# jumerckx/Monodepth2.jl

Measured on AMD Instinct MI355X. Metric: train-step images/sec, ResNet-18 416×128; 1/2/4/8 MI355X + roofline %, higher is better.
Workload: dtype fp32; 1 GPU; train_step resnet18 depth+pose decoders, 4-scale photometric loss, ADAM; batch_per_gpu=12, global_batch=12, height=128, width=416, parallelism=dp1

## Files before the change

monodepth2.jl_amd/csrc/conv_impl.inc:

```
#include <type_traits>

#include "conv.h"
#include "head.h"

namespace md2 {

typedef float f32x16 __attribute__((ext_vector_type(16)));

constexpr int KPAD = 32;
constexpr int MPAD = 128;

static inline long round_up(long a, long b) { return (a + b - 1) / b * b; }

__device__ __forceinline__ int refl(int i, int n) { return i < 0 ? -i : (i >= n ? 2 * n - 2 - i : i); }

__device__ __forceinline__ float apply_act(float v, int act) {
  switch (act) {
    case ACT_RELU: return fmaxf(v, 0.f);
    case ACT_ELU: return v > 0.f ? v : expm1f(v);
    case ACT_SIGMOID: return 1.f / (1.f + expf(-v));
    default: return v;
  }
}

// ... 156 lines not shown
  }
}

__global__ __launch_bounds__(256) void pack_batch_kernel(const PackJob* __restrict__ jobs, int njobs) {
  __shared__ int s_job;
  if (threadIdx.x == 0) {
    int lo = 0, hi = njobs - 1;
    while (lo < hi) {
      const int mid = (lo + hi + 1) >> 1;
      if (jobs[mid].block_begin <= (long)blockIdx.x) lo = mid; else hi = mid - 1;
    }
    s_job = lo;
  }
  __syncthreads();
  const PackJob& j = jobs[__builtin_amdgcn_readfirstlane(s_job)];
  if (j.tiled) {
    pack_tile(j, (int)(blockIdx.x - j.block_begin));
    return;
  }
  const unsigned e = (unsigned)(blockIdx.x - j.block_begin) * 256u + threadIdx.x;
  const unsigned KK = (unsigned)j.KK, Cinw = (unsigned)j.Cinw;
  if (e >= (unsigned)j.Cout * Cinw * KK) return;
  const float v = j.w[e];
  const unsigned row = e / KK;
  const int tap = (int)(e - row * KK);
  const int co = (int)(row / Cinw);
  const int ci = (int)(row - (unsigned)co * Cinw);
  if (j.f.out) {
    const int k = j.f.tap ? tap * j.Cin + ci : ci * j.KK + tap;
    pack_store(j.f.out, k, co, j.f.layout, j.f.Mpad, v);
  }
  if (j.d.out) {
    const int k = j.d.tap ? tap * j.Cout + co : co * j.KK + tap;
    pack_store(j.d.out, k, ci, j.d.layout, j.d.Mpad, v);
  }
}

int& conv_arith_ref() {
  static thread_local int v = 1;
  return v;
}
int conv_last_arith() { return conv_arith_ref(); }

int conv_pack_batch(const PackJob* dev_jobs, int njobs, long total_blocks, hipStream_t st) {
  if (njobs == 0) return MD2_OK;
  hipLaunchKernelGGL(pack_batch_kernel, dim3(total_blocks), dim3(256), 0, st, dev_jobs, njobs);
  MD2_LAUNCH_CHECK();
  return MD2_OK;
}

#endif

struct GemmDims {
  int M;
  long N;
  int K;
  int kper;
  int Mpad;
};

struct ConvArgs {
  GemmDims g;
  int Cin, H, W, Cout, Ho, Wo, stride, pad;
  long HW, HoWo;
  FastDiv fd_pix;
  FastDiv fd_row;
  FastDiv fd_bdiv;
  TensorIn in;
  const float* A;
  const float* dy;
  TensorOut out;
  float* slab;
  uint32_t A_bytes, b0_bytes, b1_bytes;
  uint32_t HW4, HoWo4;
  int ph_y0, ph_x0;
  int ph_taps[16];
  int ph_S;
  int ph_y0c[4], ph_x0c[4], ph_ntc[4];
  int xcd;
  int hx_cper;
  int hx_r, hx_nchunk;
  int hx_ext;
  double* bn_part;
};

__device__ __forceinline__ void out_pixel(const ConvArgs& a, bool phase, int y0, int x0, long nn,
                                          int& img, long& pix, long& plane) {
  img = (int)fdiv((uint32_t)nn, a.fd_pix);
  const long r = nn - (long)img * a.fd_pix.d;
  if (phase) {
    const int jy = (int)fdiv((uint32_t)r, a.fd_row);
    const int jx = (int)(r - (long)jy * a.fd_row.d);
    pix = (long)(y0 + 2 * jy) * a.W + x0 + 2 * jx;
    plane = a.HW;
  } else {
    pix = r;
    plane = a.fd_pix.d;
  }
}

__device__ __forceinline__ void out_pixel(const ConvArgs& a, bool phase, long nn, int& img, long& pix,
                                          long& plane) {
  out_pixel(a, phase, a.ph_y0, a.ph_x0, nn, img, pix, plane);
}

template <int TM, int TN, int BK>
__device__ __forceinline__ void mma_chunk(const float* __restrict__ As, int lda,
                                          const float* __restrict__ Bs, int ldb, int am0, int bn0,
                                          int lane, f32x16 (&acc)[TM][TN]) {
  const int kh = lane >> 5, l = lane & 31;
  float a[2][TM], b[2][TN];
#pragma unroll
  for (int i = 0; i < TM; ++i) a[0][i] = As[kh * lda + am0 + i * 32 + l];
#pragma unroll
  for (int j = 0; j < TN; ++j) b[0][j] = Bs[kh * ldb + bn0 + j * 32 + l];
#pragma unroll
  for (int kk = 0; kk < BK / 2; ++kk) {
    const int cur = kk & 1, nxt = cur ^ 1;
    if (kk + 1 < BK / 2) {
#pragma unroll
      for (int i = 0; i < TM; ++i) a[nxt][i] = As[(2 * kk + 2 + kh) * lda + am0 + i * 32 + l];
#pragma unroll
      for (int j = 0; j < TN; ++j) b[nxt][j] = Bs[(2 * kk + 2 + kh) * ldb + bn0 + j * 32 + l];
    }
#pragma unroll
    for (int i = 0; i < TM; ++i)
#pragma unroll
      for (int j = 0; j < TN; ++j)
        acc[i][j] = __builtin_amdgcn_mfma_f32_32x32x2f32(a[cur][i], b[cur][j], acc[i][j], 0, 0, 0);
  }
}

__device__ __forceinline__ void store_out(const TensorOut& o, int m, int img, long pix, long HoWo,
                                          float v) {
  if (o.bias) v += o.bias[m];
  v = apply_act(v, o.act);
  float* dst = (m < o.c0) ? o.p0 + (long)img * o.bs0 + (long)m * HoWo + pix
                          : o.p1 + (long)img * o.bs1 + (long)(m - o.c0) * HoWo + pix;
  if (o.accumulate)
    *dst += v;
  else
    *dst = v;
}

#include "conv_px.inc"
#include "conv_px2.inc"
#include "conv_px16.inc"
#include "conv_px3.inc"
#include "conv_wpx3.inc"

constexpr int HX_PX = 736;
constexpr int HX_PLANE = HX_PX * 32;
constexpr int HX_PAD = 16;
constexpr int HS2_PX = 416;
constexpr int HS2_PLANE = HS2_PX * 32;
int halo_launch(int mode, const ConvArgs& a, int items, int splits, int reflect, hipStream_t st);
int halo2d_launch(int mode, const ConvArgs& a, int mw, int splits, int reflect, hipStream_t st);
int halo_s2_launch(const ConvArgs& a, int items, int splits, hipStream_t st);
int whalo_launch(const ConvArgs& a, int items, int ksteps, int splits, hipStream_t st);
int& conv_arith_ref();
bool stem_s2d_applies(const ConvShape& s, const TensorIn& x, const TensorOut& y);
int stem_s2d_launch(const ConvShape& s, const ConvArgs& a, hipStream_t st);
bool stem_wgrad_s2d_applies(const ConvShape& s, const TensorIn& x);
int stem_wgrad_blocks(const ConvShape& s);
int stem_wgrad_s2d_launch(const ConvShape& s, const ConvArgs& a, hipStream_t st);

template <int P_ = 0>
__global__ __launch_bounds__(256) void splitk_reduce_px4_kernel(ConvArgs a, int splits) {
  const long idx = 4 * ((long)blockIdx.x * 256 + threadIdx.x);
  const long total = (long)a.g.M * a.g.N;
  if (idx >= total) return;
  const int m = (int)(idx / a.g.N);
  const long nn = idx - (long)m * a.g.N;
  float4 v = make_float4(0.f, 0.f, 0.f, 0.f);
#pragma unroll 4
  for (int s = 0; s < splits; ++s) {
    const float4 t = *reinterpret_cast<const float4*>(a.slab + (long)s * total + idx);
    v.x += t.x; v.y += t.y; v.z += t.z; v.w += t.w;
  }
  const TensorOut& o = a.out;
  const int img = (int)fdiv((uint32_t)nn, a.fd_pix);
  const long pix = nn - (long)img * a.fd_pix.d, HoWo = a.fd_pix.d;
  float r[4] = {v.x, v.y, v.z, v.w};
#pragma unroll
  for (int q = 0; q < 4; ++q) {
    if (o.bias) r[q] += o.bias[m];
    r[q] = apply_act(r[q], o.act);
  }
  float* dst = (m < o.c0) ? o.p0 + (long)img * o.bs0 + (long)m * HoWo + pix
                          : o.p1 + (long)img * o.bs1 + (long)(m - o.c0) * HoWo + pix;
  float4 w = make_float4(r[0], r[1], r[2], r[3]);
  if (o.accumulate) {
    const float4 d = *reinterpret_cast<const float4*>(dst);
    w.x = d.x + w.x; w.y = d.y + w.y; w.z = d.z + w.z; w.w = d.w + w.w;
  }
  *reinterpret_cast<float4*>(dst) = w;
}

template <int P_ = 0>
__global__ __launch_bounds__(256) void splitk_reduce_px_kernel(ConvArgs a, int splits, int phase, FastDiv fdN,
                                                               FastDiv fdT) {
  uint32_t idx = blockIdx.x * 256u + threadIdx.x;
  const uint32_t total = fdT.d;
  int cls = 0, y0 = a.ph_y0, x0 = a.ph_x0;
  if (phase && a.ph_S > 0) {
    cls = (int)fdiv(idx, fdT);
    if (cls >= 4) return;
    idx -= (uint32_t)cls * total;
    y0 = a.ph_y0c[cls];
    x0 = a.ph_x0c[cls];
  } else if (idx >= total) {
    return;
  }
  const int m = (int)fdiv(idx, fdN);
  const uint32_t nn = idx - (uint32_t)m * fdN.d;
  const float* p = a.slab + (size_t)cls * splits * total + idx;
  float v = 0.f;
  int s = 0;
  for (; s + 3 < splits; s += 4) {
    const float t0 = p[(size_t)s * total], t1 = p[(size_t)(s + 1) * total];
    const float t2 = p[(size_t)(s + 2) * total], t3 = p[(size_t)(s + 3) * total];
    v += t0;
    v += t1;
    v += t2;
    v += t3;
  }
  for (; s < splits; ++s) v += p[(size_t)s * total];
  int img;
  long pix, plane;
  out_pixel(a, phase != 0, y0, x0, (long)nn, img, pix, plane);
  store_out(a.out, m, img, pix, plane, v);
}

template <bool SMALL>
__global__ __launch_bounds__(256) void fold_reflect_kernel(const float* __restrict__ src, int splits, long ss,
                                                           long sn, long sc, TensorOut o, FastDiv fd_hw,
                                                           FastDiv fd_w, FastDiv fd_c, uint32_t total) {
  constexpr int NR = SMALL ? 3 : 2;
  const uint32_t idx = blockIdx.x * 256u + threadIdx.x;
  if (idx >= total) return;
  const int H = (int)fd_hw.d / (int)fd_w.d, W = (int)fd_w.d, P = W + 2;
  const uint32_t nc = fdiv(idx, fd_hw);
// ... 640 lines not shown

namespace {

constexpr int TARGET_BLOCKS = 1536;

enum TileCfg { T128x128 = 0, T64x256 = 1, T32x256 = 2, T64x128 = 3, T128x64 = 4, T64x64 = 5, T32x128 = 6,
               T128x64q = 7 };
const int TILE_BM[] = {128, 64, 32, 64, 128, 64, 32, 128};
const int TILE_BN[] = {128, 256, 256, 128, 64, 64, 128, 64};

int env_int(const char* name, int dflt) { return tuning_knob(name, dflt); }

struct Plan {
  int tile;
  int BM, BN, BK;
  int splits;
  int kper;
};

Plan plan_px(int M, long N, int K, bool bk32_ok = false, bool prefer32 = false) {
  static const int tile_override = env_int("MD2_PX_TILE", -1);
  static const int target = env_int("MD2_PX_TARGET", TARGET_BLOCKS);
  Plan p{};
  p.tile = M > 32 ? T64x64 : T32x128;
  if (tile_override >= 0 && tile_override <= T128x64q &&
      ((M > 32 && TILE_BM[tile_override] >= 64) || (M <= 32 && TILE_BM[tile_override] == 32)))
    p.tile = tile_override;
  p.BM = TILE_BM[p.tile];
  p.BN = TILE_BN[p.tile];
  static const int bk_override = env_int("MD2_PX_BK", 0);
  p.BK = ((bk_override == 32 || (prefer32 && bk_override != 16)) && bk32_ok) ? 32 : 16;
  if (K <= 0) {
    p.splits = 1;
    p.kper = p.BK;
    return p;
  }
  static const int minch = std::max(1, env_int("MD2_PX_MINCH", 8));
  const long tiles = (long)cdiv(M, p.BM) * cdiv(N, p.BN);
  int splits = 1;
  while (tiles * splits * 2 <= target && K / (splits * 2) >= minch * p.BK) splits *= 2;
  p.kper = (int)round_up(cdiv(K, splits), p.BK);
  p.splits = cdiv(K, p.kper);
  return p;
}

struct HaloPlan {
  bool ok = false;
  int items = 0, splits = 1, cper = 1;
  bool d2 = false;
  int mw = 2;
};
HaloPlan plan_halo(const ConvShape& s, int mode) {
  HaloPlan h;
  static const int on = env_int("MD2_HALO", 1);
  static const int target = env_int("MD2_HX_TARGET", 256);
  if (!on || mode > 1 || s.KH != 3 || s.KW != 3 || s.stride != 1 || s.pad != 1 || (s.reflect && mode == 1)) return h;
  if (!conv_px3_used(s, mode) || !conv_tap_major(s, mode)) return h;
  const int M = mode == 0 ? s.Cout : s.Cin, C = mode == 0 ? s.Cin : s.Cout;
  if (C % 16 || s.cin_w) return h;
  const int hrmax = 255 / s.W + 4;
  const bool flat = M % 64 == 0 && hrmax * (s.W + HX_PAD) + 3 <= HX_PX && cdiv((long)hrmax * s.W, 512) <= 2;
  static const int d2on = env_int("MD2_HALO2D", 1);
  const bool d2 = !flat && (d2on >> mode & 1) && M % 32 == 0 && tuning_knob("MD2_PX3_TERMS", 6) != 9 &&
                  2L * s.H * s.W >= (long)round_up(s.H, 8) * round_up(s.W, 32);
  if (!flat && !d2) return h;
  long tiles;
  int tgt = target;
  if (flat) {
    h.items = cdiv((long)hrmax * s.W, 512);
    tiles = (long)(M / 64) * cdiv((long)s.N * s.H * s.W, 256);
  } else {
    h.d2 = true;
    h.mw = M % 64 == 0 ? 2 : 1;
    tiles = (long)(M / (32 * h.mw)) * s.N * cdiv(s.H, 8) * cdiv(s.W, 32);
    tgt = h.mw == 1 ? 2 * target : target;
  }
  const int nch = C / 16;
  int splits = 1;
  while (tiles * splits * 2 <= tgt && nch / (splits * 2) >= 2) splits *= 2;
  h.cper = cdiv(nch, splits);
  h.splits = cdiv(nch, h.cper);
  h.ok = true;
  return h;
}

struct HaloS2Plan {
  bool ok = false;
  int items = 0, splits = 1, cper = 1;
};
HaloS2Plan plan_halo_s2(const ConvShape& s) {
  HaloS2Plan h;
  static const int on = env_int("MD2_HALO_S2", 1);
  if (!on || s.KH != 3 || s.KW != 3 || s.stride != 2 || s.pad != 1 || s.reflect || s.cin_w) return h;
  if (s.H != 2 * s.Ho || s.W != 2 * s.Wo || s.Cin % 64 || s.Cout % 16) return h;
  if (!conv_px3_used(s, 1) || !conv_tap_major(s, 1) || tuning_knob("MD2_PX3_TERMS", 6) == 9) return h;
  const int hrmax = 127 / s.Wo + 4;
  if (hrmax * (s.Wo + HX_PAD) + 3 > HS2_PX) return h;
  h.items = 1;
  const long tiles = (long)(s.Cin / 64) * cdiv((long)s.N * s.Ho * s.Wo, 128);
  const int nch = s.Cout / 16;
  int splits = 1;
  while (tiles * splits * 2 <= 256 && nch / (splits * 2) >= 2) splits *= 2;
  h.cper = cdiv(nch, splits);
  h.splits = cdiv(nch, h.cper);
  h.ok = true;
  return h;
}

struct WHaloPlan {
  bool ok = false;
  int r = 0, items = 0, nchunk = 0, splits = 1, cper = 1;
};
WHaloPlan plan_whalo(const ConvShape& s, int c0) {
  WHaloPlan h;
  static const int on = env_int("MD2_WHALO", 1);
  static const int target = env_int("MD2_WHX_TARGET", 256);
  if (!on || s.KH != 3 || s.KW != 3 || s.stride != 1 || s.pad != 1 || s.reflect) return h;
  if (s.Cin % 32 || s.Cout % 64 || c0 < s.Cin || (s.cin_w && s.cin_w != s.Cin) || s.W > 112) return h;
  if (tuning_knob("MD2_PX3_TERMS", 6) == 9) return h;
  int r = 0;
  for (int d = 1; d <= s.H; ++d)
    if (s.H % d == 0 && d * s.W <= 112) r = d;
  if (r == 0 || (r * s.W) % 4 || (s.H * s.W) % 4 || r * s.W < 49) return h;
  if (3L * (((r + 2) * (s.W + 2) + 3) * 64) + 448 > 65536) return h;
  static const int maxit = env_int("MD2_WHX_MAXITEMS", 4);
  h.items = cdiv(4L * (r + 2) * s.W, 384);
  if (h.items > std::min(4, maxit)) return h;
  h.r = r;
  h.nchunk = s.N * s.H / r;
  const long tiles = (long)(s.Cin / 32) * (s.Cout / 64);
  long splits = std::max(1L, (long)target / tiles);
  splits = std::min(splits, std::max(1L, (long)h.nchunk / 2));
  h.cper = cdiv(h.nchunk, splits);
  h.splits = cdiv(h.nchunk, h.cper);
  h.ok = true;
  return h;
}

ConvShape reflect_ext_shape(const ConvShape& s) {
  ConvShape e = s;
  e.H = s.H + 2;
  e.W = s.W + 2;
  e.Ho = e.H;
  e.Wo = e.W;
  e.reflect = 0;
  return e;
}
bool reflect_dgrad_on_halo(const ConvShape& s, HaloPlan* hp = nullptr) {
  static const int on = env_int("MD2_HALO_RFL_DGRAD", 1);
  if (!on || !s.reflect || s.KH != 3 || s.stride != 1 || s.pad != 1 || s.cin_w || s.H < 2 || s.W < 2) return false;
  const HaloPlan h = plan_halo(reflect_ext_shape(s), 1);
  if (hp) *hp = h;
  return h.ok;
}
size_t reflect_dgrad_ws(const ConvShape& s) {
  HaloPlan h;
  if (!reflect_dgrad_on_halo(s, &h)) return 0;
  const long Ne = (long)s.N * (s.H + 2) * (s.W + 2);
  return ((size_t)(h.splits > 1 ? h.splits : 0) + 1) * s.Cin * Ne * sizeof(float);
}

enum WTileCfg { W64x128 = 0, W32x256 = 1, W64x64 = 2, W32x128 = 3, W16x144 = 4, WSTEM = 5, W64x192 = 6 };
const int WT_BM[] = {64, 32, 64, 32, 16, 64, 64};
const int WT_BN[] = {128, 256, 64, 128, 144, 64, 192};

struct WPlan {
// ... 101 lines not shown

int check_shape(const ConvShape& s) {
  MD2_CHECK_ARG(s.N > 0 && s.Cin > 0 && s.Cout > 0 && s.H > 0 && s.W > 0, "conv dims");
  MD2_CHECK_ARG(s.KH == s.KW && (s.KH == 1 || s.KH == 3 || s.KH == 7), "kernel size 1/3/7");
  MD2_CHECK_ARG(s.stride == 1 || s.stride == 2, "stride 1/2");
  MD2_CHECK_ARG(s.Ho == (s.H + 2 * s.pad - s.KH) / s.stride + 1 &&
                    s.Wo == (s.W + 2 * s.pad - s.KW) / s.stride + 1, "output size");
  MD2_CHECK_ARG(!s.reflect || (s.KH == 3 && s.stride == 1 && s.pad == 1 && s.H >= 2 && s.W >= 2),
                "reflect padding needs 3x3/1 pad 1");
  MD2_CHECK_ARG((long)s.N * s.H * s.W < (1L << 31) && (long)s.N * s.Ho * s.Wo < (1L << 31),
                "pixel count");
  MD2_CHECK_ARG(s.cin_w >= 0 && s.cin_w <= s.Cin && (s.cin_w == 0 || s.Cout > 1),
                "weight channels (cin_w) must be <= Cin (and no padded head convs)");
  return MD2_OK;
}

#define MD2_CONV_COMBOS(X) X(1, 1, 0) X(1, 2, 0) X(3, 1, 0) X(3, 1, 1) X(3, 2, 0) X(7, 2, 0)

static int px3_terms() {
  static const int t = tuning_knob("MD2_PX3_TERMS", 6) == 9 ? 9 : 6;
  return t;
}

template <int MODE, int BM, int BN, int WM, int WN>
int launch_px_tile(const ConvShape& s, const ConvArgs& a, bool tap, int bk, dim3 grid, hipStream_t st) {
  const bool v2 = conv_px2_used(s, MODE);
  const bool v3 = conv_px3_used(s, MODE);
#define MD2_PX_CASE(KS, SS, RR)                                                                  \
  if (s.KH == KS && s.stride == SS && s.reflect == RR) {                                         \
    if constexpr (BM >= 32 && BN % 64 == 0 && WM * WN == 4) {                                    \
      if (v3) {                                                                                  \
        conv_arith_ref() = 6;                                                                    \
        if (px3_terms() == 6)                                                                    \
          hipLaunchKernelGGL((conv_px3_kernel<MODE, BM, BN, WM, WN, KS, KS, SS, RR, 16, 6>), grid, \
                             dim3(256), 0, st, a);                                               \
        else                                                                                     \
          hipLaunchKernelGGL((conv_px3_kernel<MODE, BM, BN, WM, WN, KS, KS, SS, RR, 16, 9>), grid, \
                             dim3(256), 0, st, a);                                               \
        MD2_LAUNCH_CHECK();                                                                      \
        return MD2_OK;                                                                           \
      }                                                                                          \
    }                                                                                            \
    if constexpr (BM >= 64 && BN % 64 == 0) {                                                    \
      if (v2) {                                                                                  \
        conv_arith_ref() = 1;                                                                    \
        if (bk == 32)                                                                            \
          hipLaunchKernelGGL((conv_px2_kernel<MODE, BM, BN, WM, WN, KS, KS, SS, RR, 32>), grid,  \
                             dim3(256), 0, st, a);                                               \
        else                                                                                     \
          hipLaunchKernelGGL((conv_px2_kernel<MODE, BM, BN, WM, WN, KS, KS, SS, RR, 16>), grid,  \
                             dim3(256), 0, st, a);                                               \
        MD2_LAUNCH_CHECK();                                                                      \
        return MD2_OK;                                                                           \
      }                                                                                          \
    }                                                                                            \
    if (v2) {                                                                                    \
      set_error("conv: k-contiguous kernel needs a tile with BM >= 64");                         \
      return MD2_EINVAL;                                                                         \
    }                                                                                            \
    conv_arith_ref() = 1;                                                                        \
    if (tap && bk == 32)                                                                         \
      hipLaunchKernelGGL((conv_px_kernel<MODE, 1, BM, BN, 32, WM, WN, KS, KS, SS, RR>), grid,    \
                         dim3(256), 0, st, a);                                                   \
    else if (tap)                                                                                \
      hipLaunchKernelGGL((conv_px_kernel<MODE, 1, BM, BN, 16, WM, WN, KS, KS, SS, RR>), grid,    \
                         dim3(256), 0, st, a);                                                   \
    else                                                                                         \
      hipLaunchKernelGGL((conv_px_kernel<MODE, 0, BM, BN, 16, WM, WN, KS, KS, SS, RR>), grid,    \
                         dim3(256), 0, st, a);                                                   \
    MD2_LAUNCH_CHECK();                                                                          \
    return MD2_OK;                                                                               \
  }
  MD2_CONV_COMBOS(MD2_PX_CASE)
#undef MD2_PX_CASE
  set_error("conv: unsupported (kernel, stride, padding) combination");
  return MD2_ENOTSUP;
}

template <int MODE>
int launch_px16(const ConvShape& s, ConvArgs& a, hipStream_t st) {
  a.slab = nullptr;
  conv_arith_ref() = 1;
  a.g.kper = (int)round_up(a.g.K, 16);
  static const int bn = env_int("MD2_PX16_BN", 128);
  const bool big = bn == 256;
  const dim3 grid(cdiv(a.g.N, big ? 256 : 128));
#define MD2_P16_CASE(KS, SS, RR)                                                                 \
  if constexpr (SS == 1) {                                                                       \
    if (s.KH == KS && s.stride == SS && s.reflect == RR) {                                       \
      if (big)                                                                                   \
        hipLaunchKernelGGL((conv_px16_kernel<MODE, 256, KS, KS, SS, RR>), grid, dim3(256), 0, st, a); \
      else                                                                                       \
        hipLaunchKernelGGL((conv_px16_kernel<MODE, 128, KS, KS, SS, RR>), grid, dim3(256), 0, st, a); \
      MD2_LAUNCH_CHECK();                                                                        \
      return MD2_OK;                                                                             \
    }                                                                                            \
  }
  MD2_P16_CASE(3, 1, 0) MD2_P16_CASE(3, 1, 1)
#undef MD2_P16_CASE
  set_error("conv: 16-row kernel supports 3x3 stride 1 only");
  return MD2_ENOTSUP;
}

template <int MODE>
int launch_px(const ConvShape& s, ConvArgs& a, const Plan& p_in, ConvWorkspace ws, hipStream_t st,
              SplitKDefer* defer = nullptr) {
  double* const stats = defer ? defer->stats : nullptr;
  const bool keep_reduce = defer && defer->keep_reduce;
  if (defer) *defer = SplitKDefer{};
  if (conv_px16_used(s, MODE)) return launch_px16<MODE>(s, a, st);
  HaloPlan hp = plan_halo(s, MODE);
  if (hp.ok && MODE == 0 && (a.in.bdiv < s.N || (a.in.p1 && a.in.c0 < s.Cin && a.in.c0 % 16))) hp.ok = false;
  Plan p = p_in;
  if (hp.ok) {
    p.splits = hp.splits;
    p.kper = hp.cper * 16;
  }
  a.g.kper = p.kper;
  a.slab = nullptr;
  if (p.splits > 1) {
    const size_t need = (size_t)p.splits * a.g.M * a.g.N * sizeof(float);
    MD2_CHECK_ARG(ws.ptr && ws.bytes >= need, "conv split-K workspace too small");
    a.slab = (float*)ws.ptr;
  }
  const int ncls = (MODE == 1 && a.ph_S > 0) ? 4 : 1;
  if (ncls > 1) {
    a.ph_S = p.splits;
    MD2_CHECK_ARG(p.splits == 1 || (ws.ptr && ws.bytes >= 4 * (size_t)p.splits * a.g.M * a.g.N * sizeof(float)),
                  "conv split-K workspace too small");
  }
  dim3 grid(cdiv(a.g.N, p.BN), cdiv(a.g.M, p.BM), p.splits * ncls);
  const bool tap = conv_tap_major(s, MODE);
  int rc;
  if (hp.ok && ncls == 1) {
    a.hx_cper = hp.cper;
    const TensorOut& oo = a.out;
    const bool bnst = MODE == 0 && stats && !hp.d2 && hp.splits == 1 && !s.reflect && !oo.bias && oo.act == ACT_NONE &&
                      !oo.accumulate && oo.c0 >= a.g.M && oo.bs0 == (long)a.g.M * a.fd_pix.d;
    a.bn_part = bnst ? stats : nullptr;
    conv_arith_ref() = 6;
    rc = hp.d2 ? halo2d_launch(MODE, a, hp.mw, hp.splits, s.reflect, st)
               : halo_launch(MODE, a, hp.items, hp.splits, s.reflect, st);
    a.bn_part = nullptr;
    if (rc == MD2_OK && bnst) {
      defer->stats = stats;
      defer->stats_parts = (int)cdiv(a.g.N, 256);
    }
  } else switch (p.tile) {
    case T128x128: rc = launch_px_tile<MODE, 128, 128, 2, 2>(s, a, tap, p.BK, grid, st); break;
    case T64x256: rc = launch_px_tile<MODE, 64, 256, 1, 4>(s, a, tap, p.BK, grid, st); break;
    case T64x128: rc = launch_px_tile<MODE, 64, 128, 2, 2>(s, a, tap, p.BK, grid, st); break;
    case T128x64: rc = launch_px_tile<MODE, 128, 64, 2, 2>(s, a, tap, p.BK, grid, st); break;
    case T64x64: rc = launch_px_tile<MODE, 64, 64, 2, 2>(s, a, tap, p.BK, grid, st); break;
    case T32x128: rc = launch_px_tile<MODE, 32, 128, 1, 4>(s, a, tap, p.BK, grid, st); break;
    case T128x64q: rc = launch_px_tile<MODE, 128, 64, 4, 1>(s, a, tap, p.BK, grid, st); break;
    default: rc = launch_px_tile<MODE, 32, 256, 1, 4>(s, a, tap, p.BK, grid, st); break;
  }
  if (rc) return rc;
  const TensorOut& o = a.out;
  if (defer && !keep_reduce && p.splits > 1 && ncls == 1 && (MODE == 0 || s.stride == 1) && !o.bias && o.act == ACT_NONE &&
      !o.accumulate && o.c0 >= a.g.M && o.bs0 == (long)a.g.M * a.fd_pix.d) {
    defer->slab = a.slab;
    defer->splits = p.splits;
    return MD2_OK;
  }
  const int phase = (int)(MODE == 1 && s.stride == 2 && conv_tap_major(s, 1));
  const bool aligned4 = a.fd_pix.d % 4 == 0 && o.bs0 % 4 == 0 && (!o.p1 || o.bs1 % 4 == 0) &&
                        ((uintptr_t)o.p0 % 16) == 0 && (!o.p1 || ((uintptr_t)o.p1 % 16) == 0);
  if (p.splits > 1 && ncls == 1 && !phase && aligned4) {
    const long total4 = (long)a.g.M * a.g.N / 4;
    hipLaunchKernelGGL(splitk_reduce_px4_kernel<0>, dim3(cdiv(total4, 256)), dim3(256), 0, st, a,
                       p.splits);
    MD2_LAUNCH_CHECK();
    return MD2_OK;
  }
  if (p.splits > 1) {
    const long total = (long)a.g.M * a.g.N * ncls;
    MD2_CHECK_ARG(total < (1L << 31), "conv: split-K reduction index exceeds 2^31");
    hipLaunchKernelGGL(splitk_reduce_px_kernel<0>, dim3(cdiv(total, 256)), dim3(256), 0, st, a, p.splits,
                       (int)(MODE == 1 && s.stride == 2 && conv_tap_major(s, 1)),
                       make_fastdiv((uint32_t)a.g.N), make_fastdiv((uint32_t)((long)a.g.M * a.g.N)));
    MD2_LAUNCH_CHECK();
  }
  return MD2_OK;
}

static bool wgrad_px3_on() {
  static const int v = tuning_knob("MD2_WPX3", 1);
  return v != 0;
}

template <int BM, int BN, int WM, int WN, int KS, int SS, int RR, int CW, int PX>
// ... 553 lines not shown
    default: return g;
  }
}

__global__ __launch_bounds__(256) void act_bias_kernel(const float* __restrict__ out,
                                                       const float* __restrict__ dout,
                                                       float* __restrict__ dpre, int C, int parts,
                                                       uint32_t U, FastDiv fdq, int act,
                                                       float* __restrict__ part) {
  __shared__ float red[4];
  const int c = blockIdx.x, p = blockIdx.y;
  const uint32_t beg = (uint32_t)((unsigned long long)U * p / parts);
  const uint32_t end = (uint32_t)((unsigned long long)U * (p + 1) / parts);
  const uint32_t Q = fdq.d;
  float s = 0.f;
  constexpr int UN = 4;
  for (uint32_t u0 = beg + threadIdx.x; u0 < end; u0 += 256 * UN) {
    float4 o[UN], g[UN];
    long idx[UN];
#pragma unroll
    for (int q = 0; q < UN; ++q) {
      const uint32_t u = u0 + 256 * q;
      const uint32_t uu = u < end ? u : u0;
      const uint32_t img = fdiv(uu, fdq), k = uu - img * Q;
      idx[q] = ((long)(img * (uint32_t)C + (uint32_t)c) * Q + k) * 4;
      o[q] = *reinterpret_cast<const float4*>(out + idx[q]);
      g[q] = *reinterpret_cast<const float4*>(dout + idx[q]);
    }
#pragma unroll
    for (int q = 0; q < UN; ++q) {
      if (u0 + 256 * q >= end) break;
      float4 d;
      d.x = act_grad(o[q].x, g[q].x, act);
      d.y = act_grad(o[q].y, g[q].y, act);
      d.z = act_grad(o[q].z, g[q].z, act);
      d.w = act_grad(o[q].w, g[q].w, act);
      *reinterpret_cast<float4*>(dpre + idx[q]) = d;
      s += (d.x + d.y) + (d.z + d.w);
    }
  }
  float v[1] = {s};
  block_sum256<1>(v, red);
  if (threadIdx.x == 0) part[(long)c * parts + p] = v[0];
}

int act_bias_parts(int C, int N, long HW) {
  const long U = (long)N * HW / 4;
  return (int)std::max(1L, std::min((long)std::max(1, 2048 / C), U / 1024 + 1));
}

int act_backward_bias(const float* out, const float* dout, float* dpre, int N, int C, long HW,
                      int act, float* part, hipStream_t st) {
  MD2_CHECK_ARG(HW % 4 == 0 && (long)N * C * HW < (1L << 31), "act_backward_bias: HW % 4, size");
  const int parts = act_bias_parts(C, N, HW);
  hipLaunchKernelGGL(act_bias_kernel, dim3(C, parts), dim3(256), 0, st, out, dout, dpre, C, parts,
                     (uint32_t)((long)N * HW / 4), make_fastdiv((uint32_t)(HW / 4)), act, part);
  MD2_LAUNCH_CHECK();
  return MD2_OK;
}

int act_backward(const float* out, const float* dout, float* dpre, long n, int act,
                 hipStream_t st) {
  hipLaunchKernelGGL(act_backward_kernel, dim3(cdiv(n, 256)), dim3(256), 0, st, out, dout, dpre, n,
                     act);
  MD2_LAUNCH_CHECK();
  return MD2_OK;
}

#endif

}

#if MD2_CONV_PART == 4
namespace md2 {
#include "conv_halo.inc"
}
#endif

#if MD2_CONV_PART == 5
namespace md2 {
#include "conv_stem.inc"
}
#endif
```

Baseline: 1909 images/s.

## Add thin-channel 3x3 conv kernel with LDS halo tiles and split-bf16 MFMA

```diff
diff --git a/monodepth2.jl_amd/csrc/conv_impl.inc b/monodepth2.jl_amd/csrc/conv_impl.inc
--- a/monodepth2.jl_amd/csrc/conv_impl.inc
+++ b/monodepth2.jl_amd/csrc/conv_impl.inc
@@ -262,6 +262,7 @@
   int hx_r, hx_nchunk;
   int hx_ext;
   double* bn_part;
+  int thin_layout;
 };
 
 __device__ __forceinline__ void out_pixel(const ConvArgs& a, bool phase, int y0, int x0, long nn,
@@ -338,6 +339,8 @@
 int halo2d_launch(int mode, const ConvArgs& a, int mw, int splits, int reflect, hipStream_t st);
 int halo_s2_launch(const ConvArgs& a, int items, int splits, hipStream_t st);
 int whalo_launch(const ConvArgs& a, int items, int ksteps, int splits, hipStream_t st);
+int thin_launch(int mode, const ConvArgs& a, int mt, int nch, int reflect, hipStream_t st);
+size_t thin_lds_host(int mt, int nch);
 int& conv_arith_ref();
 bool stem_s2d_applies(const ConvShape& s, const TensorIn& x, const TensorOut& y);
 int stem_s2d_launch(const ConvShape& s, const ConvArgs& a, hipStream_t st);
@@ -1144,6 +1147,26 @@
   h.splits = cdiv(nch, h.cper);
   h.ok = true;
   return h;
+}
+
+struct ThinPlan {
+  bool ok = false;
+  int mt = 1, nch = 1, layout = 0;
+};
+ThinPlan plan_thin(const ConvShape& s, int mode) {
+  ThinPlan t;
+  static const int on = env_int("MD2_THIN", 3);
+  if (mode > 1 || !(on >> mode & 1) || s.KH != 3 || s.KW != 3 || s.stride != 1 || s.pad != 1 || s.cin_w) return t;
+  if (s.H < 2 || s.W < 2 || !conv_tap_major(s, mode)) return t;
+  const int M = mode == 0 ? s.Cout : s.Cin, C = mode == 0 ? s.Cin : s.Cout;
+  if ((M != 16 && M != 32) || (C != 16 && C != 32) || (M == 32 && C == 32)) return t;
+  if ((M == 32 || C == 32) && !(on & 4)) return t;
+  if (conv_px3_used(s, mode)) return t;
+  t.layout = (conv_px2_used(s, mode) || conv_px16_used(s, mode)) ? 1 : 0;
+  t.mt = M / 16;
+  t.nch = C / 16;
+  t.ok = true;
+  return t;
 }
 
 struct HaloS2Plan {
@@ -1411,16 +1434,11 @@
   a.slab = nullptr;
   conv_arith_ref() = 1;
   a.g.kper = (int)round_up(a.g.K, 16);
-  static const int bn = env_int("MD2_PX16_BN", 128);
-  const bool big = bn == 256;
-  const dim3 grid(cdiv(a.g.N, big ? 256 : 128));
+  const dim3 grid(cdiv(a.g.N, 128));
 #define MD2_P16_CASE(KS, SS, RR)                                                                 \
   if constexpr (SS == 1) {                                                                       \
     if (s.KH == KS && s.stride == SS && s.reflect == RR) {                                       \
-      if (big)                                                                                   \
-        hipLaunchKernelGGL((conv_px16_kernel<MODE, 256, KS, KS, SS, RR>), grid, dim3(256), 0, st, a); \
-      else                                                                                       \
-        hipLaunchKernelGGL((conv_px16_kernel<MODE, 128, KS, KS, SS, RR>), grid, dim3(256), 0, st, a); \
+      hipLaunchKernelGGL((conv_px16_kernel<MODE, 128, KS, KS, SS, RR>), grid, dim3(256), 0, st, a); \
       MD2_LAUNCH_CHECK();                                                                        \
       return MD2_OK;                                                                             \
     }                                                                                            \
@@ -1437,6 +1455,14 @@
   double* const stats = defer ? defer->stats : nullptr;
   const bool keep_reduce = defer && defer->keep_reduce;
   if (defer) *defer = SplitKDefer{};
+  if (const ThinPlan tp = plan_thin(s, MODE);
+      tp.ok && !(MODE == 0 && (a.in.bdiv < s.N || (a.in.p1 && a.in.c0 < s.Cin))) && !(MODE == 1 && a.ph_S > 0)) {
+    a.slab = nullptr;
+    a.g.kper = (int)round_up(a.g.K, 16);
+    a.thin_layout = tp.layout;
+    conv_arith_ref() = 6;
+    return thin_launch(MODE, a, tp.mt, tp.nch, s.reflect, st);
+  }
   if (conv_px16_used(s, MODE)) return launch_px16<MODE>(s, a, st);
   HaloPlan hp = plan_halo(s, MODE);
   if (hp.ok && MODE == 0 && (a.in.bdiv < s.N || (a.in.p1 && a.in.c0 < s.Cin && a.in.c0 % 16))) hp.ok = false;
@@ -2156,3 +2182,9 @@
 #include "conv_stem.inc"
 }
 #endif
+
+#if MD2_CONV_PART == 6
+namespace md2 {
+#include "conv_thin.inc"
+}
+#endif
diff --git a/monodepth2.jl_amd/csrc/conv_thin.hip b/monodepth2.jl_amd/csrc/conv_thin.hip
--- /dev/null
+++ b/monodepth2.jl_amd/csrc/conv_thin.hip
@@ -0,0 +1,2 @@
+#define MD2_CONV_PART 6
+#include "conv_impl.inc"
diff --git a/monodepth2.jl_amd/csrc/conv_thin.inc b/monodepth2.jl_amd/csrc/conv_thin.inc
--- /dev/null
+++ b/monodepth2.jl_amd/csrc/conv_thin.inc
@@ -0,0 +1,258 @@
+
+typedef float tn_f32x4 __attribute__((ext_vector_type(4)));
+
+__device__ __forceinline__ uint32_t tn_swz(uint32_t off) { return off ^ ((off >> 4) & 16u); }
+
+constexpr int TN_TW = 32, TN_PR = TN_TW + 2;
+constexpr int thin_hpx(int TH) { return (TH + 2) * TN_PR; }
+constexpr int thin_plane(int TH) { return (thin_hpx(TH) + 1) * 32; }
+constexpr int thin_a_bytes(int MT, int NCH) { return 9 * NCH * 3 * MT * 512; }
+constexpr int thin_lds_bytes(int MT, int NCH, int TH) { return NCH * 3 * thin_plane(TH) + thin_a_bytes(MT, NCH); }
+constexpr int thin_th(int NCH) { return NCH == 2 ? 4 : 8; }
+
+template <int MODE, int MT, int NCH, int RFL>
+__global__ __launch_bounds__(256) void conv_thin_kernel(ConvArgs a) {
+  constexpr int TH = thin_th(NCH);
+  constexpr int HPX = thin_hpx(TH), PLANE = thin_plane(TH);
+  constexpr int RW = TH / 4, NS = 2 * RW;
+  constexpr int A_OFF = NCH * 3 * PLANE, A_PART = MT * 512;
+  constexpr int ITEMS = HPX * NCH, ROUNDS = (ITEMS + 255) / 256;
+  static_assert(A_OFF + 9 * NCH * 3 * A_PART == thin_lds_bytes(MT, NCH, TH), "LDS layout");
+  static_assert(thin_lds_bytes(MT, NCH, TH) <= 80 * 1024, "two blocks per CU");
+  static_assert((MT == 1 || MT == 2) && (NCH == 1 || NCH == 2) && TH % 4 == 0, "class");
+  extern __shared__ __attribute__((aligned(16))) uint8_t lds[];
+
+  const int tid = threadIdx.x, lane = tid & 63;
+  const int wq = __builtin_amdgcn_readfirstlane(tid >> 6);
+  const int fi = lane & 15, fg = lane >> 4;
+  const int W = a.W, H = a.H;
+  const int tx_n = (W + TN_TW - 1) / TN_TW, ty_n = (H + TH - 1) / TH;
+  const uint32_t bt = blockIdx.x;
+  const uint32_t img = bt / (uint32_t)(tx_n * ty_n);
+  const int trem = (int)(bt - img * (uint32_t)(tx_n * ty_n));
+  const int ty = trem / tx_n, tx = trem - ty * tx_n;
+  const int y0 = ty * TH, x0 = tx * TN_TW;
+
+  constexpr int APAIRS = 9 * NCH * MT * 128, AIT = (APAIRS + 255) / 256;
+  float av[AIT][2];
+  int aoffl[AIT];
+  {
+    const __amdgpu_buffer_rsrc_t rA = make_rsrc(a.A, a.A_bytes);
+    const uint32_t Mpad = (uint32_t)a.g.Mpad;
+    const bool kcont = a.thin_layout == 1;
+#pragma unroll
+    for (int i = 0; i < AIT; ++i) {
+      const int e = tid + 256 * i;
+      const int c2 = e & 7, rr = e >> 3;
+      const int m = rr % (16 * MT), kc = rr / (16 * MT);
+      const uint32_t k = (uint32_t)(kc * 16 + 2 * c2);
+      uint32_t o0 = kcont ? (((uint32_t)kc * Mpad + (uint32_t)m) * 16u + 2u * (uint32_t)c2) * 4u
+                          : (k * Mpad + (uint32_t)m) * 4u;
+      uint32_t o1 = kcont ? o0 + 4u : o0 + Mpad * 4u;
+      aoffl[i] = kc * 3 * A_PART + (int)tn_swz((uint32_t)(m * 32 + c2 * 4));
+      if (e >= APAIRS) {
+        o0 = o1 = OOB;
+        aoffl[i] = -1;
+      }
+      av[i][0] = bload(rA, o0);
+      av[i][1] = bload(rA, o1);
+    }
+  }
+
+  const uint32_t img_stride = MODE == 0 ? (uint32_t)a.in.bs0 : (uint32_t)(a.Cout * a.HoWo);
+  const uint32_t ch4 = MODE == 0 ? a.HW4 : a.HoWo4;
+  const __amdgpu_buffer_rsrc_t rB = make_rsrc(MODE == 0 ? (const void*)a.in.p0 : (const void*)a.dy, a.b0_bytes);
+  float stg[ROUNDS][16];
+  int loff[ROUNDS];
+#pragma unroll
+  for (int r = 0; r < ROUNDS; ++r) {
+    const int it = tid + 256 * r;
+    uint32_t goff = OOB;
+    loff[r] = -1;
+    if (it < ITEMS) {
+      const int cc = NCH == 1 ? 0 : (it >= HPX ? 1 : 0);
+      const int q = it - cc * HPX;
+      const int hr = q / TN_PR, hc = q - hr * TN_PR;
+      int y = y0 + hr - 1, x = x0 + hc - 1;
+      if (MODE == 0 && RFL) {
+        y = y < 0 ? -y : (y >= H ? 2 * H - 2 - y : y);
+        x = x < 0 ? -x : (x >= W ? 2 * W - 2 - x : x);
+      }
+      if (y >= 0 && y < H && x >= 0 && x < W)
+        goff = (img * img_stride + (uint32_t)(y * W + x)) * 4u + (uint32_t)(cc * 16) * ch4;
+      loff[r] = cc * 3 * PLANE + (int)tn_swz((uint32_t)q * 32u);
+    }
+#pragma unroll
+    for (int ch = 0; ch < 16; ++ch) stg[r][ch] = bload_s(rB, goff, (uint32_t)ch * ch4);
+  }
+
+  if (tid < NCH * 3 * 2)
+    *reinterpret_cast<u32x4_t*>(lds + (tid >> 1) * PLANE + HPX * 32 + (tid & 1) * 16) = u32x4_t{0u, 0u, 0u, 0u};
+#pragma unroll
+  for (int i = 0; i < AIT; ++i) {
+    if (aoffl[i] < 0) continue;
+    uint32_t h, md, l;
+    split3_pk(av[i][0], av[i][1], h, md, l);
+    uint8_t* dst = lds + A_OFF + aoffl[i];
+    *reinterpret_cast<uint32_t*>(dst) = h;
+    *reinterpret_cast<uint32_t*>(dst + A_PART) = md;
+    *reinterpret_cast<uint32_t*>(dst + 2 * A_PART) = l;
+  }
+#pragma unroll
+  for (int r = 0; r < ROUNDS; ++r) {
+    if (loff[r] < 0) continue;
+    uint32_t hm[3][8];
+#pragma unroll
+    for (int p = 0; p < 8; ++p) split3_pk(stg[r][2 * p], stg[r][2 * p + 1], hm[0][p], hm[1][p], hm[2][p]);
+#pragma unroll
+    for (int q = 0; q < 3; ++q) {
+      uint8_t* dst = lds + q * PLANE;
+      *reinterpret_cast<u32x4_t*>(dst + loff[r]) = u32x4_t{hm[q][0], hm[q][1], hm[q][2], hm[q][3]};
+      *reinterpret_cast<u32x4_t*>(dst + (loff[r] ^ 16)) = u32x4_t{hm[q][4], hm[q][5], hm[q][6], hm[q][7]};
+    }
+  }
+  __syncthreads();
+
+  int hp[NS];
+  int rflag[NS], cflag[NS];
+  bool rowb = false, colb = false;
+#pragma unroll
+  for (int s = 0; s < NS; ++s) {
+    const int row = wq * RW + (s >> 1), col = 16 * (s & 1) + fi;
+    hp[s] = (row + 1) * TN_PR + col + 1;
+    rflag[s] = cflag[s] = 0;
+    if (MODE == 1 && RFL) {
+      const int y = y0 + row, x = x0 + col;
+      if (y < H && x < W) {
+        rflag[s] = (y == 1 ? 1 : 0) | (y == H - 2 ? 2 : 0);
+        cflag[s] = (x == 1 ? 1 : 0) | (x == W - 2 ? 2 : 0);
+      }
+      rowb |= rflag[s] != 0;
+      colb |= cflag[s] != 0;
+    }
+  }
+  if (MODE == 1 && RFL) {
+    rowb = __ballot(rowb) != 0;
+    colb = __ballot(colb) != 0;
+  }
+  const int half16 = 16 * (fg & 1);
+  const int b1sel = (fg >> 1) ? PLANE : 0;
+  const int b3sel = (fg >> 1) ? 0 : 2 * PLANE;
+  const int a3sel = (fg >> 1) ? 2 * A_PART : 0;
+  int aoff[MT];
+#pragma unroll
+  for (int mi = 0; mi < MT; ++mi) aoff[mi] = (int)tn_swz((uint32_t)((mi * 16 + fi) * 32 + half16));
+
+  tn_f32x4 accb[MT][NS], accs[MT][NS];
+#pragma unroll
+  for (int mi = 0; mi < MT; ++mi)
+#pragma unroll
+    for (int s = 0; s < NS; ++s)
+#pragma unroll
+      for (int r = 0; r < 4; ++r) accb[mi][s][r] = accs[mi][s][r] = 0.f;
+
+#pragma unroll
+  for (int cc = 0; cc < NCH; ++cc) {
+    const uint8_t* bimg = lds + cc * 3 * PLANE;
+#pragma unroll
+    for (int tap = 0; tap < 9; ++tap) {
+      const int kh = tap / 3, kw = tap - 3 * kh;
+      const int dy = MODE == 0 ? kh - 1 : 1 - kh;
+      const int dx = MODE == 0 ? kw - 1 : 1 - kw;
+      const uint8_t* abase = lds + A_OFF + (tap * NCH + cc) * 3 * A_PART;
+      bf16x8_t fa[MT][3];
+#pragma unroll
+      for (int mi = 0; mi < MT; ++mi) {
+        fa[mi][0] = __builtin_bit_cast(bf16x8_t, *reinterpret_cast<const u32x4_t*>(abase + aoff[mi]));
+        fa[mi][1] = __builtin_bit_cast(bf16x8_t, *reinterpret_cast<const u32x4_t*>(abase + A_PART + aoff[mi]));
+        fa[mi][2] = __builtin_bit_cast(bf16x8_t, *reinterpret_cast<const u32x4_t*>(abase + a3sel + aoff[mi]));
+      }
+      auto taps = [&](const int (&pix)[NS]) {
+#pragma unroll
+        for (int s = 0; s < NS; ++s) {
+          const uint32_t off = tn_swz((uint32_t)pix[s] * 32u + (uint32_t)half16);
+          const bf16x8_t b1 = __builtin_bit_cast(bf16x8_t, *reinterpret_cast<const u32x4_t*>(bimg + b1sel + off));
+          const bf16x8_t b3 = __builtin_bit_cast(bf16x8_t, *reinterpret_cast<const u32x4_t*>(bimg + b3sel + off));
+#pragma unroll
+          for (int mi = 0; mi < MT; ++mi) {
+            tn_f32x4 c = accs[mi][s];
+            c = __builtin_amdgcn_mfma_f32_16x16x32_bf16(fa[mi][1], b1, c, 0, 0, 0);
+            c = __builtin_amdgcn_mfma_f32_16x16x32_bf16(fa[mi][2], b3, c, 0, 0, 0);
+            accs[mi][s] = c;
+            accb[mi][s] = __builtin_amdgcn_mfma_f32_16x16x32_bf16(fa[mi][0], b1, accb[mi][s], 0, 0, 0);
+          }
+        }
+      };
+      int pix[NS];
+#pragma unroll
+      for (int s = 0; s < NS; ++s) pix[s] = hp[s] + dy * TN_PR + dx;
+      taps(pix);
+      if constexpr (MODE == 1 && RFL != 0) {
+#pragma unroll
+        for (int combo = 1; combo < 4; ++combo) {
+          const bool ry = combo & 1, rx = combo >> 1;
+          if ((ry && kh == 1) || (rx && kw == 1)) continue;
+          if ((ry && !rowb) || (rx && !colb)) continue;
+#pragma unroll
+          for (int s = 0; s < NS; ++s) {
+            const bool ok = (!ry || ((rflag[s] >> (kh >> 1)) & 1)) && (!rx || ((cflag[s] >> (kw >> 1)) & 1));
+            pix[s] = ok ? hp[s] + (ry ? -dy : dy) * TN_PR + (rx ? -dx : dx) : HPX;
+          }
+          taps(pix);
+        }
+      }
+    }
+  }
+
+#pragma unroll
+  for (int s = 0; s < NS; ++s) {
+    const int y = y0 + wq * RW + (s >> 1), x = x0 + 16 * (s & 1) + fi;
+    if (y >= H || x >= W) continue;
+    const long pix = (long)y * W + x;
+#pragma unroll
+    for (int mi = 0; mi < MT; ++mi)
+#pragma unroll
+      for (int r = 0; r < 4; ++r)
+        store_out(a.out, mi * 16 + 4 * fg + r, (int)img, pix, (long)a.fd_pix.d, accb[mi][s][r] + accs[mi][s][r]);
+  }
+}
+
+#if MD2_CONV_PART == 6
+size_t thin_lds_host(int mt, int nch) { return (size_t)thin_lds_bytes(mt, nch, thin_th(nch)); }
+
+int thin_launch(int mode, const ConvArgs& a, int mt, int nch, int reflect, hipStream_t st) {
+  MD2_CHECK_ARG((mt == 1 || mt == 2) && (nch == 1 || nch == 2) && mt * nch <= 2, "conv_thin: class");
+  MD2_CHECK_ARG(a.g.M == 16 * mt && (mode == 0 ? a.Cin : a.Cout) == 16 * nch, "conv_thin: channels");
+  MD2_CHECK_ARG(a.thin_layout == 0 || a.thin_layout == 1, "conv_thin: packed layout");
+  const long tiles = (long)cdiv(a.W, TN_TW) * cdiv(a.H, thin_th(nch));
+  const long blocks = a.g.N / ((long)a.H * a.W) * tiles;
+  MD2_CHECK_ARG(blocks > 0 && blocks < (1L << 31), "conv_thin: grid");
+  const dim3 grid((unsigned)blocks);
+  const size_t lds = thin_lds_host(mt, nch);
+#define MD2_TN_LAUNCH(MO, MTV, NCHV, RR)                                                          \
+  {                                                                                              \
+    constexpr size_t need = (size_t)thin_lds_bytes(MTV, NCHV, thin_th(NCHV));                    \
+    MD2_CHECK_ARG(lds >= need, "conv_thin: dynamic LDS smaller than the kernel's image");        \
+    static bool attr = false;                                                                    \
+    if (!attr) {                                                                                 \
+      MD2_HIP(hipFuncSetAttribute((const void*)conv_thin_kernel<MO, MTV, NCHV, RR>,              \
+                                  hipFuncAttributeMaxDynamicSharedMemorySize, (int)need));      \
+      attr = true;                                                                               \
+    }                                                                                            \
+    hipLaunchKernelGGL((conv_thin_kernel<MO, MTV, NCHV, RR>), grid, dim3(256), lds, st, a);      \
+  }
+#define MD2_TN_CLASS(MO, RR)                                                                     \
+  if (mt == 1 && nch == 1) MD2_TN_LAUNCH(MO, 1, 1, RR)                                           \
+  else if (mt == 2) MD2_TN_LAUNCH(MO, 2, 1, RR)                                                  \
+  else MD2_TN_LAUNCH(MO, 1, 2, RR)
+  if (mode == 0) {
+    if (reflect) { MD2_TN_CLASS(0, 1) } else { MD2_TN_CLASS(0, 0) }
+  } else {
+    if (reflect) { MD2_TN_CLASS(1, 1) } else { MD2_TN_CLASS(1, 0) }
+  }
+#undef MD2_TN_CLASS
+#undef MD2_TN_LAUNCH
+  MD2_LAUNCH_CHECK();
+  return MD2_OK;
+}
+#endif
```

Result: no change. 1924 images/s, median of 6 (+0.8%).
